# NVIDIA-Merlin/NVTabular

Measured on AMD Instinct MI355X. Metric: rows/sec + GB/s (Criteo Categorify+FillMissing+Normalize fit+transform, HBM-resident), higher is better.
Workload: dtype int32 keys -> int64 labels; fp64 moments/normalize; 1 GPU; synthetic Criteo-day0: 26 int32 categorical (Criteo-1TB cardinalities, Zipf) + 13 int32 continuous, nulls as Arrow bitmaps; Categorify + FillMissing + Normalize, fit + transform; rows_per_gpu=45000000, algorithmic_bytes_per_row=624, tie_break=value (count desc, value asc), artifacts=deferred (no parquet I/O inside the timed region)

## Files before the change

nvtabular_amd/csrc/nvt_encode.hip:

```cpp
#include <cstdlib>
#include <limits>
#include <type_traits>

#include "nvt_common.hpp"
#include "nvt_internal.hpp"
#include "nvt_prof.hpp"
#include "nvt_range.hpp"

namespace nvt {

template <typename K>
struct EncSlot;
template <>
struct EncSlot<int32_t> {
  int32_t key;
  int32_t label;
};
template <>
struct EncSlot<int64_t> {
  int64_t key;
  int64_t label;
};
template <typename K>
struct EncTraits;
// ... 20 lines not shown
  for (uint64_t i = (uint64_t)blockIdx.x * kBlock + threadIdx.x; i < capacity; i += stride)
    table[i] = e;
  if (blockIdx.x == 0 && threadIdx.x == 0) *sentinel_label = -1;
}

template <typename K>
__global__ __launch_bounds__(kBlock) void enc_build_kernel(const K *__restrict__ vocab, uint64_t n,
                                                           int64_t first_label, EncSlot<K> *table,
                                                           uint64_t mask, int64_t *sentinel_label) {
  constexpr K EMPTY = EncTraits<K>::empty;
  using C = typename EncTraits<K>::cas_t;
  const uint64_t stride = (uint64_t)gridDim.x * kBlock;
  for (uint64_t i = (uint64_t)blockIdx.x * kBlock + threadIdx.x; i < n; i += stride) {
    K key = vocab[i];
    int64_t label = first_label + (int64_t)i;
    if (key == EMPTY) {
      atomicMin(reinterpret_cast<unsigned long long *>(sentinel_label), (unsigned long long)label);
      continue;
    }
    uint64_t slot = (uint64_t)slot_hash(key) & mask;
    while (true) {
      K prev = (K)atomicCAS(reinterpret_cast<C *>(&table[slot].key), (C)EMPTY, (C)key);
      if (prev == EMPTY || prev == key) {
        using L = decltype(table[slot].label);
        if constexpr (sizeof(L) == 4)
          atomicMin(reinterpret_cast<int *>(&table[slot].label), (int)label);
        else
          atomicMin(reinterpret_cast<long long *>(&table[slot].label), (long long)label);
        break;
      }
      slot = (slot + 1) & mask;
    }
  }
}

__global__ __launch_bounds__(kBlock) void enc_build_unique_i32_kernel(
    const int32_t *__restrict__ vocab, uint64_t n, int64_t first_label, EncSlot<int32_t> *table,
    uint64_t mask, int64_t *sentinel_label) {
  const unsigned long long EMPTY_SLOT =
      ((unsigned long long)(uint32_t)std::numeric_limits<int32_t>::max() << 32) |
      (unsigned long long)(uint32_t)INT32_MIN;
  const uint64_t stride = (uint64_t)gridDim.x * kBlock;
  for (uint64_t i = (uint64_t)blockIdx.x * kBlock + threadIdx.x; i < n; i += stride) {
    int32_t key = vocab[i];
    int64_t label = first_label + (int64_t)i;
    if (key == INT32_MIN) {
      *sentinel_label = label;
      continue;
    }
    unsigned long long want = ((unsigned long long)(uint32_t)label << 32) | (uint32_t)key;
    uint64_t slot = (uint64_t)slot_hash(key) & mask;
    while (atomicCAS(reinterpret_cast<unsigned long long *>(&table[slot]), EMPTY_SLOT, want) !=
           EMPTY_SLOT)
      slot = (slot + 1) & mask;
  }
}

template <typename K>
__device__ __forceinline__ int64_t probe(const EncSlot<K> *__restrict__ table, uint64_t mask,
                                         K key) {
  constexpr K EMPTY = EncTraits<K>::empty;
  uint64_t slot = (uint64_t)slot_hash(key) & mask;
  while (true) {
    EncSlot<K> s = table[slot];
    if (s.key == key) return (int64_t)s.label;
    if (s.key == EMPTY) return -1;
    slot = (slot + 1) & mask;
  }
}

template <typename K, typename OUT>
__global__ __launch_bounds__(kBlock) void encode_kernel(
    const K *__restrict__ keys, const uint8_t *__restrict__ valid, uint64_t n,
    const EncSlot<K> *__restrict__ table, uint64_t mask, const int64_t *__restrict__ sentinel_label,
    int64_t null_label, int64_t oov_label, uint32_t num_buckets, OUT *__restrict__ out) {
  constexpr K EMPTY = EncTraits<K>::empty;
  constexpr int VEC = EncTraits<K>::vec;
  const int64_t sent = *sentinel_label;

  auto label_of = [&](K key, bool ok) -> OUT {
    if (!ok) return (OUT)null_label;
    int64_t lab = (key == EMPTY) ? sent : probe<K>(table, mask, key);
    if (lab < 0) {
      lab = oov_label;
      if (num_buckets > 1) lab += (int64_t)(key_hash32((int64_t)key) % num_buckets);
    }
    return (OUT)lab;
  };

  const uint64_t nvec = n / VEC;
  const uint64_t stride = (uint64_t)gridDim.x * kBlock;
  using VecT = typename std::conditional<sizeof(K) == 4, int4, longlong2>::type;
  const VecT *vkeys = reinterpret_cast<const VecT *>(keys);
  for (uint64_t v = (uint64_t)blockIdx.x * kBlock + threadIdx.x; v < nvec; v += stride) {
    VecT pack = vkeys[v];
    unsigned vbits = 0xF;
    if (valid != nullptr) {
      uint64_t row = v * VEC;
      vbits = (valid[row >> 3] >> (row & 7));
    }
    K k[VEC];
    if constexpr (sizeof(K) == 4) {
      k[0] = pack.x;
      k[1] = pack.y;
      k[2] = pack.z;
      k[3] = pack.w;
    } else {
      k[0] = pack.x;
      k[1] = pack.y;
    }
    OUT r[VEC];
#pragma unroll
    for (int j = 0; j < VEC; ++j) r[j] = label_of(k[j], (vbits >> j) & 1);
    OUT *dst = out + v * VEC;
    if constexpr (VEC * sizeof(OUT) == 32) {
      int4 a, b;
      memcpy(&a, &r[0], 16);
      memcpy(&b, &r[2], 16);
      reinterpret_cast<int4 *>(dst)[0] = a;
      reinterpret_cast<int4 *>(dst)[1] = b;
    } else if constexpr (VEC * sizeof(OUT) == 16) {
      int4 a;
      memcpy(&a, &r[0], 16);
      reinterpret_cast<int4 *>(dst)[0] = a;
    } else {
      int2 a;
      memcpy(&a, &r[0], 8);
      reinterpret_cast<int2 *>(dst)[0] = a;
    }
  }
  for (uint64_t i = nvec * VEC + (uint64_t)blockIdx.x * kBlock + threadIdx.x; i < n; i += stride)
    out[i] = label_of(keys[i], bit_valid(valid, i));
}

typedef int nvt_v4i __attribute__((ext_vector_type(4)));
template <typename V>
__device__ __forceinline__ V nt_load16(const V *p) {
  static_assert(sizeof(V) == 16, "16-byte vectors only");
  nvt_v4i r = __builtin_nontemporal_load(reinterpret_cast<const nvt_v4i *>(p));
  V v;
  memcpy(&v, &r, 16);
  return v;
}
template <typename V>
__device__ __forceinline__ void nt_store16(V v, V *p) {
  static_assert(sizeof(V) == 16, "16-byte vectors only");
  nvt_v4i r;
  memcpy(&r, &v, 16);
  __builtin_nontemporal_store(r, reinterpret_cast<nvt_v4i *>(p));
}
#ifndef NVT_HOT_DIV
#define NVT_HOT_DIV 4
#endif
constexpr int kEncBS = 1024;
template <typename K>
struct HotCfg;
template <>
struct HotCfg<int32_t> {
  static constexpr int slots = 16384;
};
template <>
struct HotCfg<int64_t> {
  static constexpr int slots = 8192;
};

constexpr int kHead16Buckets = 12288;
constexpr int kHead16Keys = kHead16Buckets * 2 / 8 * 7;
__device__ __forceinline__ void two_buckets16(int32_t key, uint32_t &b1, uint32_t &b2) {
  const uint32_t k = (uint32_t)key, lo = k ^ (k >> 7), hi = k >> 8;
  const uint32_t h1 = ((__umul24(hi, 0x5BD1E9u) + __umul24(lo, 0x9E3779u)) >> 17) & 0x7FFFu;
  const uint32_t h2 = ((__umul24(hi, 0x7FEB35u) + __umul24(lo, 0x846CA7u)) >> 17) & 0x7FFFu;
  b1 = (h1 + 2u * h1) >> 3;
  b2 = (h2 + 2u * h2) >> 3;
  b2 = b2 == b1 ? (b1 ^ 1u) : b2;
}
__device__ unsigned long long g_enc_stats[2];

template <int SLOTS, typename K>
__device__ __forceinline__ uint32_t lds_home(K key) {
  if constexpr (sizeof(K) == 4) {
    static_assert(SLOTS <= 16384, "14 index bits");
    return (mul24_hash((int32_t)key) >> 18) & (SLOTS - 1);
  } else {
    return (uint32_t)(slot_hash(key) >> 13) & (SLOTS - 1);
  }
}

struct HeadJob {
  const int32_t *keys;
  unsigned char *image;
  int64_t first_label;
  uint32_t n_hot;
};
constexpr int kHeadJobsMax = 32;
struct HeadJobs {
  HeadJob j[kHeadJobsMax];
};

template <typename K, bool TWO>
__device__ __forceinline__ void build_head(unsigned char *lraw, long long *s_sent_p,
                                           const K *__restrict__ hot_keys, uint32_t n_hot,
                                           int64_t first_label) {
  constexpr K EMPTY = EncTraits<K>::empty;
  constexpr int SLOTS = HotCfg<K>::slots;
  using L = decltype(EncSlot<K>::label);
  using C = typename EncTraits<K>::cas_t;
  EncSlot<K> *lt = reinterpret_cast<EncSlot<K> *>(lraw);
  int2 *tkeys = reinterpret_cast<int2 *>(lraw);
  uint32_t *tlab = reinterpret_cast<uint32_t *>(lraw + kHead16Buckets * 8);
  long long &s_sent = *s_sent_p;
  if constexpr (TWO) {
    for (int i = threadIdx.x; i < kHead16Buckets; i += kEncBS) {
      tkeys[i] = make_int2((int)EMPTY, (int)EMPTY);
      tlab[i] = 0u;
    }
  } else {
    for (int i = threadIdx.x; i < SLOTS; i += kEncBS) {
      lt[i].key = EMPTY;
      lt[i].label = 0;
    }
  }
  if (threadIdx.x == 0) s_sent = -1;
  __syncthreads();
  for (uint32_t i = threadIdx.x; i < n_hot; i += kEncBS) {
    K key = hot_keys[i];
    if (key == EMPTY) {
      s_sent = first_label + (long long)i;
      continue;
    }
    if constexpr (TWO) {
      uint32_t b1, b2;
      two_buckets16((int32_t)key, b1, b2);
      const uint32_t cand[4] = {2 * b1, 2 * b1 + 1, 2 * b2, 2 * b2 + 1};
      int *kw = reinterpret_cast<int *>(tkeys);
      unsigned short *lw = reinterpret_cast<unsigned short *>(tlab);
#pragma unroll
      for (int c = 0; c < 4; ++c) {
        const int prev = atomicCAS(&kw[cand[c]], (int)EMPTY, (int)key);
        if (prev == (int)EMPTY) {
          lw[cand[c]] = (unsigned short)i;
          break;
        }
      }
      continue;
    }
    uint32_t s = lds_home<SLOTS>(key);
    while (true) {
      K prev = (K)atomicCAS(reinterpret_cast<C *>(&lt[s].key), (C)EMPTY, (C)key);
      if (prev == EMPTY || prev == key) {
        if (prev == EMPTY) lt[s].label = (L)(first_label + (int64_t)i);
        break;
      }
      s = (s + 1) & (SLOTS - 1);
    }
  }
  __syncthreads();
}

template <typename K, bool TWO>
constexpr int kHeadLdsBytes = TWO ? kHead16Buckets * 12 : HotCfg<K>::slots * (int)sizeof(EncSlot<K>);

__global__ __launch_bounds__(kEncBS) void enc_head_build_many_kernel(HeadJobs jobs) {
  constexpr int kLdsBytes = kHeadLdsBytes<int32_t, true>;
  __shared__ __align__(16) unsigned char lraw[kLdsBytes];
  __shared__ long long s_sent;
  const HeadJob j = jobs.j[blockIdx.x];
  build_head<int32_t, true>(lraw, &s_sent, j.keys, j.n_hot, j.first_label);
  const int4 *src = reinterpret_cast<const int4 *>(lraw);
  int4 *dst = reinterpret_cast<int4 *>(j.image);
  for (int i = threadIdx.x; i < kLdsBytes / 16; i += kEncBS) dst[i] = src[i];
  if (threadIdx.x == 0) *reinterpret_cast<long long *>(j.image + kLdsBytes) = s_sent;
}

template <int SLOTS>
__global__ __launch_bounds__(kBlock) void encode_small_kernel(
    const int32_t *__restrict__ keys, const uint8_t *__restrict__ valid, uint64_t n, int64_t null_label,
    int64_t oov_label, uint32_t num_buckets, int64_t *__restrict__ out,
    const int32_t *__restrict__ hot_keys, uint32_t n_hot, int64_t first_label) {
  constexpr int32_t EMPTY = EncTraits<int32_t>::empty;
  __shared__ EncSlot<int32_t> lt[SLOTS];
  __shared__ long long s_sent;
  for (int i = threadIdx.x; i < SLOTS; i += kBlock) {
    lt[i].key = EMPTY;
    lt[i].label = 0;
  }
  if (threadIdx.x == 0) s_sent = -1;
  __syncthreads();
  for (uint32_t i = threadIdx.x; i < n_hot; i += kBlock) {
    const int32_t key = hot_keys[i];
    if (key == EMPTY) {
      s_sent = first_label + (long long)i;
      continue;
    }
    uint32_t sl = lds_home<SLOTS>(key);
    while (true) {
      const int32_t prev = atomicCAS(&lt[sl].key, EMPTY, key);
      if (prev == EMPTY || prev == key) {
        if (prev == EMPTY) lt[sl].label = (int32_t)(first_label + (int64_t)i);
        break;
      }
      sl = (sl + 1) & (SLOTS - 1);
    }
  }
  __syncthreads();
  const int64_t sent = (int64_t)s_sent;
  auto encode = [&](int32_t key, bool ok) -> int64_t {
    if (!ok) return null_label;
    int64_t lab = -1;
    if (key == EMPTY) {
      lab = sent;
    } else {
      uint32_t sl = lds_home<SLOTS>(key);
      while (true) {
        const EncSlot<int32_t> e = lt[sl];
        if (e.key == key) {
          lab = (int64_t)e.label;
          break;
        }
        if (e.key == EMPTY) break;
        sl = (sl + 1) & (SLOTS - 1);
      }
    }
    if (lab < 0) {
      lab = oov_label;
      if (num_buckets > 1) lab += (int64_t)(key_hash32((int64_t)key) % num_buckets);
    }
    return lab;
  };
  constexpr int RUN = 2 * kWave, U = 4;
  typedef int v2i_nt __attribute__((ext_vector_type(2)));
  const uint64_t stride = (uint64_t)gridDim.x * kBlock;
  const unsigned lane = threadIdx.x & (kWave - 1);
  const uint64_t nruns = n / RUN;
  const uint64_t wave = (uint64_t)blockIdx.x * (kBlock / kWave) +
                        (uint64_t)__builtin_amdgcn_readfirstlane(threadIdx.x / kWave);
  const uint64_t nwaves = stride / kWave;
  for (uint64_t r0 = wave * U; r0 < nruns; r0 += nwaves * U) {
    v2i_nt raw[U];
    unsigned vb[U];
#pragma unroll
    for (int u = 0; u < U; ++u) {
      raw[u] = v2i_nt{0, 0};
      vb[u] = 3u;
      if (r0 + u < nruns) {
        const uint64_t e = (r0 + u) * RUN + 2 * lane;
        raw[u] = __builtin_nontemporal_load(reinterpret_cast<const v2i_nt *>(keys + e));
        if (valid != nullptr) vb[u] = (unsigned)valid[e >> 3] >> (e & 7);
      }
    }
#pragma unroll
    for (int u = 0; u < U; ++u) {
      if (r0 + u >= nruns) break;
      const uint64_t e = (r0 + u) * RUN + 2 * lane;
      int64_t r[2];
      r[0] = encode(raw[u].x, (bool)(vb[u] & 1));
      r[1] = encode(raw[u].y, (bool)((vb[u] >> 1) & 1));
      nvt_v4i o;
      memcpy(&o, r, 16);
      __builtin_nontemporal_store(o, reinterpret_cast<nvt_v4i *>(out + e));
    }
  }
  for (uint64_t i = nruns * RUN + (uint64_t)blockIdx.x * kBlock + threadIdx.x; i < n; i += stride)
    out[i] = encode(keys[i], bit_valid(valid, i));
}

template <typename K, typename OUT, bool TWO = false, bool GLOBAL = true>
__global__ __launch_bounds__(kEncBS, 1) void encode_hot_kernel(
    const K *__restrict__ keys, const uint8_t *__restrict__ valid, uint64_t n,
    const EncSlot<K> *__restrict__ table, uint64_t mask, const int64_t *__restrict__ sentinel_label,
    int64_t null_label, int64_t oov_label, uint32_t num_buckets, OUT *__restrict__ out,
    const K *__restrict__ hot_keys, uint32_t n_hot, int64_t first_label, int count_stats = 0,
    const unsigned char *__restrict__ head_image = nullptr) {
  static_assert(!TWO || (GLOBAL && sizeof(K) == 4), "TWO: the 2-choice head of int32 keys in cache mode");
  constexpr bool global_needed = GLOBAL;
  constexpr K EMPTY = EncTraits<K>::empty;
  constexpr int VEC = EncTraits<K>::vec;
  constexpr int SLOTS = HotCfg<K>::slots;
  constexpr int kLdsBytes = kHeadLdsBytes<K, TWO>;
  __shared__ __align__(16) unsigned char lraw[kLdsBytes];
  EncSlot<K> *lt = reinterpret_cast<EncSlot<K> *>(lraw);
  int2 *tkeys = reinterpret_cast<int2 *>(lraw);
  uint32_t *tlab = reinterpret_cast<uint32_t *>(lraw + kHead16Buckets * 8);
  __shared__ long long s_sent;
  if (head_image != nullptr) {
    const int4 *src = reinterpret_cast<const int4 *>(head_image);
    int4 *dst = reinterpret_cast<int4 *>(lraw);
    for (int i = threadIdx.x; i < kLdsBytes / 16; i += kEncBS) dst[i] = src[i];
    if (threadIdx.x == 0) s_sent = *reinterpret_cast<const long long *>(head_image + kLdsBytes);
    __syncthreads();
  } else {
    build_head<K, TWO>(lraw, &s_sent, hot_keys, n_hot, first_label);
  }
  const int64_t sent = global_needed ? *sentinel_label : (int64_t)s_sent;

  auto hot_lookup = [&](K key) -> int64_t {
    if constexpr (TWO) {
      uint32_t b1, b2;
      two_buckets16((int32_t)key, b1, b2);
      const int2 a = tkeys[b1], c = tkeys[b2];
      const uint32_t la = tlab[b1], lc = tlab[b2];
      int lab = -1;
      lab = a.x == (int)key ? (int)(la & 0xFFFFu) : lab;
      lab = a.y == (int)key ? (int)(la >> 16) : lab;
      lab = c.x == (int)key ? (int)(lc & 0xFFFFu) : lab;
      lab = c.y == (int)key ? (int)(lc >> 16) : lab;
      return lab < 0 ? (int64_t)-1 : first_label + (int64_t)lab;
    }
    uint32_t s = lds_home<SLOTS>(key);
    while (true) {
      EncSlot<K> e = lt[s];
      if (e.key == key) return (int64_t)e.label;
      if (e.key == EMPTY) return -1;
      s = (s + 1) & (SLOTS - 1);
    }
  };
  auto finish = [&](K key, int64_t lab) -> OUT {
    if (lab < 0) {
      lab = oov_label;
      if (num_buckets > 1) lab += (int64_t)(key_hash32((int64_t)key) % num_buckets);
    }
    return (OUT)lab;
  };

  const uint64_t nvec = n / VEC;
  const uint64_t stride = (uint64_t)gridDim.x * kEncBS;
  using VecT = typename std::conditional<sizeof(K) == 4, int4, longlong2>::type;
  const VecT *vkeys = reinterpret_cast<const VecT *>(keys);
  constexpr int U = 2;
  constexpr int NK = U * VEC;
  VecT nxt_pack[U];
  unsigned nxt_vb[U];
  unsigned st_miss = 0, st_rows = 0;
  auto issue_loads = [&](uint64_t v0, VecT (&pk)[U], unsigned (&bits)[U]) {
#pragma unroll
    for (int u = 0; u < U; ++u) {
      uint64_t v = v0 + (uint64_t)u * stride;
      bits[u] = 0;
      if (v < nvec) {
        pk[u] = nt_load16(&vkeys[v]);
        bits[u] = 0x10000u | (valid ? (unsigned)valid[(v * VEC) >> 3] : 0xFFu);
      }
    }
  };
  issue_loads((uint64_t)blockIdx.x * kEncBS + threadIdx.x, nxt_pack, nxt_vb);
  for (uint64_t v0 = (uint64_t)blockIdx.x * kEncBS + threadIdx.x; v0 < nvec; v0 += stride * U) {
    VecT pack[U];
    unsigned vb[U];
#pragma unroll
    for (int u = 0; u < U; ++u) {
      pack[u] = nxt_pack[u];
      vb[u] = nxt_vb[u];
    }
    issue_loads(v0 + stride * U, nxt_pack, nxt_vb);
#pragma unroll
    for (int u = 0; u < U; ++u)
      if (vb[u])
        vb[u] = 0x100u | (((vb[u] & 0xFFu) >> (((v0 + (uint64_t)u * stride) * VEC) & 7)) &
                          ((1u << VEC) - 1u));
    K k[NK];
    int64_t lab[NK];
    bool need[NK];
#pragma unroll
    for (int u = 0; u < U; ++u) {
      if constexpr (sizeof(K) == 4) {
        k[u * VEC + 0] = pack[u].x;
        k[u * VEC + 1] = pack[u].y;
        k[u * VEC + 2] = pack[u].z;
        k[u * VEC + 3] = pack[u].w;
      } else {
        k[u * VEC + 0] = pack[u].x;
        k[u * VEC + 1] = pack[u].y;
      }
    }
#pragma unroll
    for (int q = 0; q < NK; ++q) {
      const bool ok = (vb[q / VEC] & 0x100) && ((vb[q / VEC] >> (q % VEC)) & 1);
      lab[q] = -1;
      need[q] = false;
      if (ok) {
        if (k[q] == EMPTY) {
          lab[q] = sent;
        } else {
          lab[q] = hot_lookup(k[q]);
          need[q] = lab[q] < 0 && global_needed;
          if (count_stats) {
            st_rows += 1u;
            st_miss += need[q] ? 1u : 0u;
          }
        }
      } else {
        lab[q] = null_label;
      }
    }
    if constexpr (GLOBAL) {
      uint64_t slot[NK];
      EncSlot<K> e[NK];
#pragma unroll
      for (int q = 0; q < NK; ++q) {
        slot[q] = (uint64_t)slot_hash(k[q]) & mask;
        if (need[q]) e[q] = table[slot[q]];
      }
#pragma unroll
      for (int q = 0; q < NK; ++q) {
        if (!need[q]) continue;
        while (true) {
          if (e[q].key == k[q]) {
            lab[q] = (int64_t)e[q].label;
            break;
          }
          if (e[q].key == EMPTY) break;
          slot[q] = (slot[q] + 1) & mask;
          e[q] = table[slot[q]];
        }
      }
    }
#pragma unroll
    for (int u = 0; u < U; ++u) {
      if (!(vb[u] & 0x100)) continue;
      uint64_t v = v0 + (uint64_t)u * stride;
      OUT r[VEC];
#pragma unroll
      for (int j = 0; j < VEC; ++j) {
        const int q = u * VEC + j;
        const bool ok = (vb[u] >> j) & 1;
        r[j] = ok ? finish(k[q], lab[q]) : (OUT)null_label;
      }
      OUT *dst = out + v * VEC;
      if constexpr (VEC * sizeof(OUT) == 32) {
        int4 a, b;
        memcpy(&a, &r[0], 16);
        memcpy(&b, &r[2], 16);
        nt_store16(a, &reinterpret_cast<int4 *>(dst)[0]);
        nt_store16(b, &reinterpret_cast<int4 *>(dst)[1]);
      } else if constexpr (VEC * sizeof(OUT) == 16) {
        int4 a;
        memcpy(&a, &r[0], 16);
        nt_store16(a, &reinterpret_cast<int4 *>(dst)[0]);
      } else {
        int2 a;
        memcpy(&a, &r[0], 8);
        reinterpret_cast<int2 *>(dst)[0] = a;
      }
    }
  }
  for (uint64_t i = nvec * VEC + (uint64_t)blockIdx.x * kEncBS + threadIdx.x; i < n; i += stride) {
    K key = keys[i];
    OUT r = (OUT)null_label;
    if (bit_valid(valid, i)) {
      int64_t lab = key == EMPTY ? sent : hot_lookup(key);
      if (lab < 0 && key != EMPTY && global_needed) {
        uint64_t sl = (uint64_t)slot_hash(key) & mask;
        while (true) {
          const EncSlot<K> e1 = table[sl];
          if (e1.key == key) {
            lab = (int64_t)e1.label;
            break;
          }
          if (e1.key == EMPTY) break;
          sl = (sl + 1) & mask;
        }
      }
      r = finish(key, lab);
    }
    out[i] = r;
  }
  if (count_stats) {
#pragma unroll
    for (int off = 32; off > 0; off >>= 1) {
      st_miss += __shfl_down(st_miss, off, 64);
      st_rows += __shfl_down(st_rows, off, 64);
    }
    if (lane_id() == 0) {
      atomicAdd(&g_enc_stats[0], (unsigned long long)st_miss);
      atomicAdd(&g_enc_stats[1], (unsigned long long)st_rows);
    }
  }
}

#define NVT_GLOBAL_AS __attribute__((address_space(1)))
template <typename T>
__device__ __forceinline__ NVT_GLOBAL_AS T *uniform_gptr(T *p) {
  const uint64_t v = reinterpret_cast<uint64_t>(p);
  const uint32_t lo = __builtin_amdgcn_readfirstlane((uint32_t)v);
  const uint32_t hi = __builtin_amdgcn_readfirstlane((uint32_t)(v >> 32));
  return (NVT_GLOBAL_AS T *)(((uint64_t)hi << 32) | lo);
}
template <typename OUT, int RANGE>
__global__ __launch_bounds__(kEncBS, 1) void encode_pipe_kernel(
    const int32_t *__restrict__ keys, const uint8_t *__restrict__ valid, uint64_t n,
    const EncSlot<int32_t> *__restrict__ table, uint64_t mask,
    const int64_t *__restrict__ sentinel_label, int64_t null_label, int64_t oov_label,
    uint32_t num_buckets, OUT *__restrict__ out, const int32_t *__restrict__ hot_keys,
    uint32_t n_hot, int64_t first_label, const int32_t *__restrict__ range_aux, int count_stats,
    const unsigned char *__restrict__ head_image) {
  static_assert(RANGE == 1 || RANGE == 2, "range tables (slots and byte offsets fit 32 bits)");
  using K = int32_t;
  constexpr K EMPTY = EncTraits<K>::empty;
  constexpr int VEC = 4, U = 2, NK = U * VEC;
  constexpr int kLdsBytes = kHeadLdsBytes<K, true>;
  RangeMap rmap = load_map(range_aux);
  __shared__ uint32_t s_pieces[RANGE == 1 ? kRpPwWords : 1];
  if constexpr (RANGE == 1) stage_pieces(rmap, s_pieces, threadIdx.x, kEncBS);
  __shared__ __align__(16) unsigned char lraw[kLdsBytes];
  const int2 *tkeys = reinterpret_cast<const int2 *>(lraw);
  const uint32_t *tlab = reinterpret_cast<const uint32_t *>(lraw + kHead16Buckets * 8);
  __shared__ long long s_sent;
  __shared__ unsigned s_next;
  if (threadIdx.x == 0) s_next = 0;
  if (head_image != nullptr) {
    const int4 *src = reinterpret_cast<const int4 *>(head_image);
    int4 *dst = reinterpret_cast<int4 *>(lraw);
    for (int i = threadIdx.x; i < kLdsBytes / 16; i += kEncBS) dst[i] = src[i];
    __syncthreads();
  } else {
    build_head<K, true>(lraw, &s_sent, hot_keys, n_hot, first_label);
  }
  const int32_t sent = (int32_t)*sentinel_label;
  const unsigned long long *tw = reinterpret_cast<const unsigned long long *>(table);
  const char *tbytes = reinterpret_cast<const char *>(table);

  unsigned st_miss = 0, st_rows = 0;
  auto run = [&](auto pw_tag) {
    constexpr bool PW = decltype(pw_tag)::value;
    auto first_slot = [&](K key) -> uint32_t {
      const uint32_t f = rmap.template fine_staged<PW>(key);
      return RANGE == 2 ? f : f + (f >> 14) * (uint32_t)kRpTail;
    };
    auto hot_lookup = [&](K key) -> int32_t {
      uint32_t b1, b2;
      two_buckets16(key, b1, b2);
      const int2 a = tkeys[b1], c = tkeys[b2];
      const uint32_t la = tlab[b1], lc = tlab[b2];
      int lab = -1;
      lab = a.x == key ? (int)(la & 0xFFFFu) : lab;
      lab = a.y == key ? (int)(la >> 16) : lab;
      lab = c.x == key ? (int)(lc & 0xFFFFu) : lab;
      lab = c.y == key ? (int)(lc >> 16) : lab;
      return lab < 0 ? -1 : (int32_t)first_label + lab;
    };
    auto walk = [&](K key, uint32_t sl0, unsigned long long e0) -> int32_t {
      if constexpr (RANGE == 2) {
        unsigned long long w = 0;
        const uint64_t at = flat_find_from(tw, mask + 1, (uint64_t)sl0, key, e0, &w);
        return at == ~0ull ? -1 : (int32_t)(w >> 32);
      } else {
        uint64_t sl = sl0;
        while (true) {
          const unsigned long long e = tw[++sl];
          if ((int32_t)(uint32_t)e == key) return (int32_t)(e >> 32);
          if ((int32_t)(uint32_t)e == EMPTY) return -1;
        }
      }
    };
    auto finish = [&](K key, int32_t lab) -> OUT {
      int64_t r = (int64_t)lab;
      if (lab < 0) {
        r = oov_label;
        if (num_buckets > 1) r += (int64_t)(key_hash32((int64_t)key) % num_buckets);
      }
      return (OUT)r;
    };
    auto encode_one = [&](K key, bool ok) -> OUT {
      if (!ok) return (OUT)null_label;
      int32_t lab = key == EMPTY ? sent : hot_lookup(key);
      if (lab < 0 && key != EMPTY) {
        const uint32_t sl = first_slot(key);
        const unsigned long long e = tw[sl];
        if ((int32_t)(uint32_t)e == key) lab = (int32_t)(e >> 32);
        else if ((int32_t)(uint32_t)e != EMPTY) lab = walk(key, sl, e);
      }
      return finish(key, lab);
    };

    const uint64_t nvec = n / VEC;
    const uint64_t stride = (uint64_t)gridDim.x * kEncBS, SU = stride * U;
    const uint64_t vb0 = (uint64_t)blockIdx.x * kEncBS;
    const int4 *vkeys = reinterpret_cast<const int4 *>(keys);
    const uint8_t *vsrc = valid != nullptr ? valid : reinterpret_cast<const uint8_t *>(keys);
    const unsigned vor = valid != nullptr ? 0u : 0xFFu;
    uint64_t nfull = 0;
    if (nvec >= vb0 + (uint64_t)(U - 1) * stride + kEncBS)
      nfull = (nvec - (vb0 + (uint64_t)(U - 1) * stride + kEncBS)) / SU + 1;
    const unsigned tid = threadIdx.x, lane = lane_id();
    const unsigned nib = (tid & 1u) * 4u;
    int4 nxt_pack[U];
    unsigned nxt_vb[U];
    struct Stage {
      int32_t k[NK];
      int32_t lab[NK];
      unsigned long long e[NK];
      unsigned need;
      unsigned vb[U];
    };
    auto batch_base = [&](uint64_t j, int u) -> uint64_t {
      return vb0 + (j >> 4) * SU + (uint64_t)u * stride + (j & 15u) * (uint64_t)kWave;
    };
    auto request_keys = [&](uint64_t j) {
#pragma unroll
      for (int u = 0; u < U; ++u) {
        const uint64_t vs = batch_base(j, u);
        const nvt_v4i raw = __builtin_nontemporal_load(
            reinterpret_cast<const NVT_GLOBAL_AS nvt_v4i *>(uniform_gptr(vkeys + vs)) + lane);
        nxt_pack[u] = make_int4(raw.x, raw.y, raw.z, raw.w);
        nxt_vb[u] = (unsigned)uniform_gptr(vsrc + (vs >> 1))[lane >> 1];
      }
    };
    auto lds_phase = [&](Stage &st) {
      unsigned need = 0;
#pragma unroll
      for (int u = 0; u < U; ++u) {
        st.k[u * VEC + 0] = nxt_pack[u].x;
        st.k[u * VEC + 1] = nxt_pack[u].y;
        st.k[u * VEC + 2] = nxt_pack[u].z;
        st.k[u * VEC + 3] = nxt_pack[u].w;
        st.vb[u] = ((nxt_vb[u] | vor) >> nib) & 0xFu;
      }
#pragma unroll
      for (int q = 0; q < NK; ++q) {
        const K key = st.k[q];
        const bool ok = (st.vb[q / VEC] >> (q % VEC)) & 1u;
        const bool is_sent = key == EMPTY;
        int32_t lab = hot_lookup(key);
        lab = is_sent ? sent : lab;
        st.lab[q] = lab;
        need |= ((ok & !is_sent & (lab < 0)) ? 1u : 0u) << q;
      }
      st.need = need;
      if (count_stats) {
        st_rows += (unsigned)__popc(st.vb[0]) + (unsigned)__popc(st.vb[1]);
        st_miss += (unsigned)__popc(need);
      }
    };
    auto request_probes = [&](Stage &st) {
#pragma unroll
      for (int q = 0; q < NK; ++q) {
        const uint32_t off = ((st.need >> q) & 1u) ? first_slot(st.k[q]) * 8u : 0u;
        st.e[q] = *reinterpret_cast<const unsigned long long *>(tbytes + off);
        if constexpr (PW) __builtin_amdgcn_sched_barrier(0);
      }
    };
    auto resolve = [&](Stage &st) {
      unsigned more = 0;
#pragma unroll
      for (int q = 0; q < NK; ++q) {
        const bool nd = (st.need >> q) & 1u;
        const int32_t ek = (int32_t)(uint32_t)st.e[q];
        const bool hit = nd & (ek == st.k[q]);
        st.lab[q] = hit ? (int32_t)(st.e[q] >> 32) : st.lab[q];
        more |= ((nd & !hit & (ek != EMPTY)) ? 1u : 0u) << q;
      }
      while (more) {
        const int q = (int)__ffs((int)more) - 1;
        more &= more - 1u;
        K key = st.k[0];
        unsigned long long e0 = st.e[0];
#pragma unroll
        for (int j = 1; j < NK; ++j) {
          key = q == j ? st.k[j] : key;
          e0 = q == j ? st.e[j] : e0;
        }
        const int32_t lab = walk(key, first_slot(key), e0);
#pragma unroll
        for (int j = 0; j < NK; ++j) st.lab[j] = q == j ? lab : st.lab[j];
      }
    };
    auto store = [&](const Stage &st, uint64_t j) {
#pragma unroll
      for (int u = 0; u < U; ++u) {
// ... 111 lines not shown
  if (count_stats) {
#pragma unroll
    for (int off = 32; off > 0; off >>= 1) {
      st_miss += __shfl_down(st_miss, off, 64);
      st_rows += __shfl_down(st_rows, off, 64);
    }
    if (lane_id() == 0) {
      atomicAdd(&g_enc_stats[0], (unsigned long long)st_miss);
      atomicAdd(&g_enc_stats[1], (unsigned long long)st_rows);
    }
  }
}

template <typename K>
__global__ __launch_bounds__(kBlock) void hash_bucket_kernel(const K *__restrict__ keys,
                                                             const uint8_t *__restrict__ valid,
                                                             uint64_t n, uint32_t nb,
                                                             int32_t *__restrict__ out,
                                                             const uint64_t *__restrict__ xor_in,
                                                             uint64_t *__restrict__ xor_out) {
  const uint64_t stride = (uint64_t)gridDim.x * kBlock;
  for (uint64_t i = (uint64_t)blockIdx.x * kBlock + threadIdx.x; i < n; i += stride) {
    uint64_t h = key_hash64(bit_valid(valid, i) ? (int64_t)keys[i] : 0);
    if (xor_in) h ^= xor_in[i];
    if (xor_out) xor_out[i] = h;
    if (out) out[i] = (int32_t)((uint32_t)(h >> 32) % nb);
  }
}

template <typename K>
__global__ __launch_bounds__(kBlock) void hash_bucket_vec_kernel(const K *__restrict__ keys,
                                                                 const uint8_t *__restrict__ valid,
                                                                 uint64_t n, uint32_t nb,
                                                                 int32_t *__restrict__ out) {
  constexpr int VEC = EncTraits<K>::vec;
  const uint64_t nvec = n / VEC;
  const uint64_t stride = (uint64_t)gridDim.x * kBlock;
  using VecT = typename std::conditional<sizeof(K) == 4, int4, longlong2>::type;
  const VecT *vkeys = reinterpret_cast<const VecT *>(keys);
  for (uint64_t v = (uint64_t)blockIdx.x * kBlock + threadIdx.x; v < nvec; v += stride) {
    VecT pack = vkeys[v];
    if (valid != nullptr) {
      const uint64_t row = v * VEC;
      const unsigned vb = (unsigned)valid[row >> 3] >> (row & 7);
      if (!(vb & 1)) pack.x = 0;
      if (!(vb & 2)) pack.y = 0;
      if constexpr (sizeof(K) == 4) {
        if (!(vb & 4)) pack.z = 0;
        if (!(vb & 8)) pack.w = 0;
      }
    }
    if constexpr (sizeof(K) == 4) {
      int4 r;
      r.x = (int32_t)(key_hash32(pack.x) % nb);
      r.y = (int32_t)(key_hash32(pack.y) % nb);
      r.z = (int32_t)(key_hash32(pack.z) % nb);
      r.w = (int32_t)(key_hash32(pack.w) % nb);
      reinterpret_cast<int4 *>(out)[v] = r;
    } else {
      int2 r;
      r.x = (int32_t)(key_hash32(pack.x) % nb);
      r.y = (int32_t)(key_hash32(pack.y) % nb);
      reinterpret_cast<int2 *>(out)[v] = r;
    }
  }
  for (uint64_t i = nvec * VEC + (uint64_t)blockIdx.x * kBlock + threadIdx.x; i < n; i += stride)
    out[i] = (int32_t)(key_hash32(bit_valid(valid, i) ? (int64_t)keys[i] : 0) % nb);
}

template <typename K>
int build_launch(const K *vocab, uint64_t n, int64_t first_label, void *table, uint64_t capacity,
                 int64_t *sentinel_label, int unique_keys, hipStream_t s) {
  NVT_CHECK_ARG(table && sentinel_label, "null table");
  NVT_CHECK_ARG(capacity >= 64 && (capacity & (capacity - 1)) == 0, "capacity must be 2^k >= 64");
  NVT_CHECK_ARG(capacity > n, "capacity must exceed the vocabulary size");
  NVT_CHECK_ARG(sizeof(K) == 8 || first_label + (int64_t)n < INT32_MAX, "labels overflow int32");
  NVT_CHECK_ARG(first_label >= 0, "first_label must not be negative");
  auto *t = reinterpret_cast<EncSlot<K> *>(table);
  NVT_PROF("encode_build", 0, s);
  enc_clear_kernel<K><<<stream_grid(capacity, kBlock * 4), kBlock, 0, s>>>(t, capacity,
                                                                           sentinel_label);
  NVT_CHECK_LAUNCH();
  if (n) {
    NVT_CHECK_ARG(vocab, "null vocabulary");
    if constexpr (sizeof(K) == 4) {
      if (unique_keys) {
        enc_build_unique_i32_kernel<<<stream_grid(n, kBlock), kBlock, 0, s>>>(
            vocab, n, first_label, t, capacity - 1, sentinel_label);
        NVT_CHECK_LAUNCH();
        return NVT_OK;
      }
    }
    enc_build_kernel<K><<<stream_grid(n, kBlock), kBlock, 0, s>>>(vocab, n, first_label, t,
                                                                  capacity - 1, sentinel_label);
    NVT_CHECK_LAUNCH();
  }
  return NVT_OK;
}

template <typename K>
int encode_launch(const K *keys, const uint8_t *valid, uint64_t n, const void *table,
                  uint64_t capacity, const int64_t *sentinel_label, int64_t null_label,
                  int64_t oov_label, uint32_t num_buckets, void *out, int out_bytes,
                  const K *hot_keys, uint64_t n_vocab, int64_t first_label, hipStream_t s,
                  const int32_t *range_aux = nullptr, const void *head_image = nullptr) {
  constexpr uint64_t kResident = sizeof(K) == 4 ? NVT_ENCODE_RESIDENT_I32 : NVT_ENCODE_RESIDENT_I64;
  const bool resident = hot_keys != nullptr && n_vocab > 0 && n_vocab <= kResident;
  NVT_CHECK_ARG(resident || (table && sentinel_label), "null table");
  NVT_CHECK_ARG(resident || range_aux || (capacity >= 64 && (capacity & (capacity - 1)) == 0),
                "capacity must be 2^k >= 64");
  NVT_CHECK_ARG(range_aux == nullptr || (sizeof(K) == 4 && hot_keys != nullptr && n_vocab > 0),
                "range tables: int32 keys with the ordered vocabulary (vocab_keys)");
  NVT_CHECK_ARG(out_bytes == 4 || out_bytes == 8, "out_bytes must be 4 or 8");
  if (n == 0) return NVT_OK;
  NVT_CHECK_ARG(keys && out, "null keys/out");
  NVT_CHECK_ARG((reinterpret_cast<uintptr_t>(keys) & 15) == 0 &&
                    (reinterpret_cast<uintptr_t>(out) & 15) == 0,
                "keys/out must be 16-byte aligned");
  constexpr int VEC = EncTraits<K>::vec;
  auto *t = reinterpret_cast<const EncSlot<K> *>(table);
  NVT_PROF(sizeof(K) == 4 ? "encode_i32" : "encode_i64", n * (sizeof(K) + (uint64_t)out_bytes), s);
  auto with_out = [&](auto launch) {
    if (out_bytes == 8) launch(reinterpret_cast<int64_t *>(out));
    else launch(reinterpret_cast<int32_t *>(out));
  };
  if (hot_keys != nullptr && n_vocab > 0) {
    const unsigned hgrid = stream_grid(n / VEC + 1, kEncBS * 2, 1);
    const uint64_t mask = capacity - 1;
    if (resident) {
      const uint32_t n_hot = (uint32_t)n_vocab;
      if constexpr (sizeof(K) == 4) {
        if (out_bytes == 8 && n_vocab <= 2048) {
          const unsigned sgrid = stream_grid(n / 2 + 1, kBlock * 8, 8);
          if (n_vocab <= 1024)
            encode_small_kernel<2048><<<sgrid, kBlock, 0, s>>>(
                keys, valid, n, null_label, oov_label, num_buckets, reinterpret_cast<int64_t *>(out),
                hot_keys, n_hot, first_label);
          else
            encode_small_kernel<4096><<<sgrid, kBlock, 0, s>>>(
                keys, valid, n, null_label, oov_label, num_buckets, reinterpret_cast<int64_t *>(out),
                hot_keys, n_hot, first_label);
          NVT_CHECK_LAUNCH();
          return NVT_OK;
        }
      }
      with_out([&](auto *o) {
        using OUT = std::remove_pointer_t<decltype(o)>;
        encode_hot_kernel<K, OUT, false, false><<<hgrid, kEncBS, 0, s>>>(
            keys, valid, n, t, mask, sentinel_label, null_label, oov_label, num_buckets, o, hot_keys,
            n_hot, first_label);
      });
    } else if constexpr (sizeof(K) == 4) {
      const uint32_t n_hot = (uint32_t)(n_vocab < (uint64_t)kHead16Keys ? n_vocab : (uint64_t)kHead16Keys);
      static const int stats = getenv("NVT_ENC_STATS") ? atoi(getenv("NVT_ENC_STATS")) : 0;
      const auto *image = reinterpret_cast<const unsigned char *>(head_image);
      with_out([&](auto *o) {
        using OUT = std::remove_pointer_t<decltype(o)>;
        if (range_aux == nullptr)
          encode_hot_kernel<K, OUT, true, true><<<hgrid, kEncBS, 0, s>>>(
              keys, valid, n, t, mask, sentinel_label, null_label, oov_label, num_buckets, o, hot_keys,
              n_hot, first_label, stats, image);
        else if (capacity > 0)
          encode_pipe_kernel<OUT, 2><<<hgrid, kEncBS, 0, s>>>(
              keys, valid, n, t, mask, sentinel_label, null_label, oov_label, num_buckets, o, hot_keys,
              n_hot, first_label, range_aux, stats, image);
        else
          encode_pipe_kernel<OUT, 1><<<hgrid, kEncBS, 0, s>>>(
              keys, valid, n, t, mask, sentinel_label, null_label, oov_label, num_buckets, o, hot_keys,
              n_hot, first_label, range_aux, stats, image);
      });
    } else {
      const uint32_t n_hot = (uint32_t)HotCfg<K>::slots / NVT_HOT_DIV;
      with_out([&](auto *o) {
        using OUT = std::remove_pointer_t<decltype(o)>;
        encode_hot_kernel<K, OUT, false, true><<<hgrid, kEncBS, 0, s>>>(
            keys, valid, n, t, mask, sentinel_label, null_label, oov_label, num_buckets, o, hot_keys,
            n_hot, first_label);
      });
    }
    NVT_CHECK_LAUNCH();
    return NVT_OK;
  }
  unsigned grid = stream_grid(n / VEC + 1, kBlock * 2, 8);
  if (out_bytes == 8)
    encode_kernel<K, int64_t><<<grid, kBlock, 0, s>>>(keys, valid, n, t, capacity - 1,
                                                      sentinel_label, null_label, oov_label,
                                                      num_buckets, reinterpret_cast<int64_t *>(out));
  else
    encode_kernel<K, int32_t><<<grid, kBlock, 0, s>>>(keys, valid, n, t, capacity - 1,
                                                      sentinel_label, null_label, oov_label,
                                                      num_buckets, reinterpret_cast<int32_t *>(out));
  NVT_CHECK_LAUNCH();
  return NVT_OK;
}

template <typename K>
int hash_bucket_launch(const K *keys, const uint8_t *valid, uint64_t n, uint32_t nb, int32_t *out,
                       const uint64_t *xor_in, uint64_t *xor_out, hipStream_t s) {
  NVT_CHECK_ARG(nb >= 1 && nb < (1u << 31), "num_buckets must be in [1, 2^31)");
  if (n == 0) return NVT_OK;
  NVT_CHECK_ARG(keys && (out || xor_out), "null keys/out");
  bool aligned = (reinterpret_cast<uintptr_t>(keys) & 15) == 0 &&
                 (reinterpret_cast<uintptr_t>(out) & 15) == 0;
  NVT_PROF("hash_bucket", n * (sizeof(K) + 4), s);
  if (!xor_in && !xor_out && aligned)
    hash_bucket_vec_kernel<K><<<stream_grid(n / EncTraits<K>::vec + 1, kBlock * 2), kBlock, 0, s>>>(
        keys, valid, n, nb, out);
  else
    hash_bucket_kernel<K><<<stream_grid(n, kBlock * 4), kBlock, 0, s>>>(keys, valid, n, nb, out,
                                                                       xor_in, xor_out);
  NVT_CHECK_LAUNCH();
  return NVT_OK;
}

int encode_build_any(int key_bytes, const void *vocab, uint64_t n, int64_t first_label, void *table,
                     uint64_t capacity, int64_t *sentinel_label, int unique_keys, hipStream_t s) {
  if (key_bytes == 4)
    return build_launch<int32_t>((const int32_t *)vocab, n, first_label, table, capacity,
                                 sentinel_label, unique_keys, s);
  return build_launch<int64_t>((const int64_t *)vocab, n, first_label, table, capacity,
                               sentinel_label, unique_keys, s);
}

int encode_clear_any(int key_bytes, void *table, uint64_t capacity, int64_t *sentinel_label,
                     hipStream_t s) {
  NVT_CHECK_ARG(table && sentinel_label, "null table");
  NVT_CHECK_ARG(capacity >= 64, "capacity must be >= 64");
  NVT_PROF("encode_build", 0, s);
  if (key_bytes == 4)
    enc_clear_kernel<int32_t><<<stream_grid(capacity, kBlock * 4), kBlock, 0, s>>>(
        reinterpret_cast<EncSlot<int32_t> *>(table), capacity, sentinel_label);
  else
    enc_clear_kernel<int64_t><<<stream_grid(capacity, kBlock * 4), kBlock, 0, s>>>(
        reinterpret_cast<EncSlot<int64_t> *>(table), capacity, sentinel_label);
  NVT_CHECK_LAUNCH();
  return NVT_OK;
}

int encode_insert_any(int key_bytes, const void *vocab, uint64_t n, int64_t first_label,
                      void *table, uint64_t capacity, int64_t *sentinel_label, hipStream_t s) {
  NVT_CHECK_ARG(key_bytes == 4, "encode_insert_any: int32 keys");
  NVT_CHECK_ARG(table && sentinel_label && (n == 0 || vocab), "null pointer");
  NVT_CHECK_ARG(first_label + (int64_t)n < INT32_MAX, "labels overflow int32");
  if (n == 0) return NVT_OK;
  NVT_PROF("encode_build", 0, s);
  enc_build_unique_i32_kernel<<<stream_grid(n, kBlock), kBlock, 0, s>>>(
      (const int32_t *)vocab, n, first_label, reinterpret_cast<EncSlot<int32_t> *>(table),
      capacity - 1, sentinel_label);
  NVT_CHECK_LAUNCH();
  return NVT_OK;
}

}

using namespace nvt;

namespace nvt {
int encode_head_build_many(const int32_t *const *vocab_keys, const uint64_t *n, const int64_t *first_label,
                           void *const *images, int count, hipStream_t s) {
  const uint64_t cap = (uint64_t)kHead16Keys;
  HeadJobs jobs;
  int m = 0;
  auto flush = [&]() -> int {
    if (m == 0) return NVT_OK;
    NVT_PROF("vocab_order", 0, s);
    enc_head_build_many_kernel<<<m, kEncBS, 0, s>>>(jobs);
    NVT_CHECK_LAUNCH();
    m = 0;
    return NVT_OK;
  };
  for (int i = 0; i < count; ++i) {
    if (images[i] == nullptr || vocab_keys[i] == nullptr || n[i] <= NVT_ENCODE_RESIDENT_I32) continue;
    jobs.j[m].keys = vocab_keys[i];
    jobs.j[m].image = (unsigned char *)images[i];
    jobs.j[m].first_label = first_label[i];
    jobs.j[m].n_hot = (uint32_t)(n[i] < cap ? n[i] : cap);
    if (++m == kHeadJobsMax) {
      int rc = flush();
      if (rc) return rc;
    }
  }
  return flush();
}
int encode_head_build(const int32_t *vocab_keys, uint64_t n, int64_t first_label, void *image,
                      hipStream_t s) {
  return encode_head_build_many(&vocab_keys, &n, &first_label, &image, 1, s);
}
}

extern "C" {

int nvt_encode_stats(uint64_t *out2, int reset, void *stream) {
  NVT_CHECK_ARG(out2, "null out");
  hipStream_t s = (hipStream_t)stream;
  NVT_CHECK_HIP(hipStreamSynchronize(s));
  unsigned long long v[2] = {0, 0};
  NVT_CHECK_HIP(hipMemcpyFromSymbol(v, HIP_SYMBOL(g_enc_stats), sizeof(v)));
  out2[0] = v[0];
  out2[1] = v[1];
  if (reset) {
    const unsigned long long z[2] = {0, 0};
    NVT_CHECK_HIP(hipMemcpyToSymbol(HIP_SYMBOL(g_enc_stats), z, sizeof(z)));
  }
  return NVT_OK;
}

int nvt_encode_table_bytes(int key_bytes, uint64_t capacity, uint64_t *bytes) {
  NVT_CHECK_ARG(bytes && (key_bytes == 4 || key_bytes == 8), "key_bytes must be 4 or 8");
  *bytes = capacity * (key_bytes == 4 ? sizeof(EncSlot<int32_t>) : sizeof(EncSlot<int64_t>));
  return NVT_OK;
}
int nvt_encode_build_i32(const int32_t *vocab_keys, uint64_t n_vocab, int64_t first_label,
                         void *table, uint64_t capacity, int64_t *sentinel_label, int unique_keys,
                         void *stream) {
  return build_launch<int32_t>(vocab_keys, n_vocab, first_label, table, capacity, sentinel_label,
                               unique_keys, (hipStream_t)stream);
}
int nvt_encode_build_i64(const int64_t *vocab_keys, uint64_t n_vocab, int64_t first_label,
                         void *table, uint64_t capacity, int64_t *sentinel_label, int unique_keys,
                         void *stream) {
  return build_launch<int64_t>(vocab_keys, n_vocab, first_label, table, capacity, sentinel_label,
                               unique_keys, (hipStream_t)stream);
}
int nvt_encode_i32(const int32_t *keys, const uint8_t *valid, uint64_t n, const void *table,
                   uint64_t capacity, const int64_t *sentinel_label, int64_t null_label,
                   int64_t oov_label, uint32_t num_buckets, void *out, int out_bytes,
                   const int32_t *vocab_keys, uint64_t n_vocab, int64_t first_label,
                   void *stream) {
  return encode_launch<int32_t>(keys, valid, n, table, capacity, sentinel_label, null_label,
                                oov_label, num_buckets, out, out_bytes, vocab_keys, n_vocab,
                                first_label, (hipStream_t)stream);
}
int nvt_encode_i64(const int64_t *keys, const uint8_t *valid, uint64_t n, const void *table,
                   uint64_t capacity, const int64_t *sentinel_label, int64_t null_label,
                   int64_t oov_label, uint32_t num_buckets, void *out, int out_bytes,
                   const int64_t *vocab_keys, uint64_t n_vocab, int64_t first_label,
                   void *stream) {
  return encode_launch<int64_t>(keys, valid, n, table, capacity, sentinel_label, null_label,
                                oov_label, num_buckets, out, out_bytes, vocab_keys, n_vocab,
                                first_label, (hipStream_t)stream);
}
int nvt_encode_many(const nvt_encode_col *cols, int ncols, void *stream) {
  NVT_CHECK_ARG(ncols == 0 || cols, "null descriptors");
  const int n_side = [] {
    const char *e = getenv("NVT_ENCODE_STREAMS");
    int v = e ? atoi(e) : 3;
    return v < 1 ? 1 : v > kSideStreams ? kSideStreams : v;
  }();
  hipStream_t main_s = (hipStream_t)stream;
  SidePool *pool = nullptr;
  const int lanes = ncols < n_side ? ncols : n_side;
  const bool fork = lanes > 1;
  if (fork) {
    int rc = side_pool(2, &pool);
    if (rc) return rc;
    NVT_CHECK_HIP(hipEventRecord(pool->fork, main_s));
    for (int k = 0; k < lanes; ++k) NVT_CHECK_HIP(hipStreamWaitEvent(pool->s[k], pool->fork, 0));
  }
  int rc_all = NVT_OK;
  for (int i = 0; i < ncols; ++i) {
    const nvt_encode_col &c = cols[i];
    hipStream_t cs = fork ? pool->s[i % lanes] : main_s;
    int rc;
    if (c.wait_event) NVT_CHECK_HIP(hipStreamWaitEvent(cs, (hipEvent_t)c.wait_event, 0));
    if (c.key_bytes == 4)
      rc = encode_launch<int32_t>((const int32_t *)c.keys, c.valid, c.n, c.table, c.capacity,
                                  c.sentinel_label, c.null_label, c.oov_label, c.num_buckets, c.out,
                                  c.out_bytes, (const int32_t *)c.vocab_keys, c.n_vocab,
                                  c.first_label, cs, c.range_aux, c.head_image);
    else if (c.key_bytes == 8)
      rc = encode_launch<int64_t>((const int64_t *)c.keys, c.valid, c.n, c.table, c.capacity,
                                  c.sentinel_label, c.null_label, c.oov_label, c.num_buckets, c.out,
                                  c.out_bytes, (const int64_t *)c.vocab_keys, c.n_vocab,
                                  c.first_label, cs);
    else {
      set_error("nvt_encode_many: key_bytes must be 4 or 8 (column %d)", i);
      rc = NVT_EINVAL;
    }
    if (rc) {
      rc_all = rc;
      break;
    }
  }
  if (fork)
    for (int k = 0; k < lanes; ++k) {
      NVT_CHECK_HIP(hipEventRecord(pool->join[k], pool->s[k]));
      NVT_CHECK_HIP(hipStreamWaitEvent(main_s, pool->join[k], 0));
    }
  return rc_all;
}
int nvt_hash_bucket_i32(const int32_t *keys, const uint8_t *valid, uint64_t n, uint32_t num_buckets,
                        int32_t *out, const uint64_t *xor_in, uint64_t *xor_out, void *stream) {
  return hash_bucket_launch<int32_t>(keys, valid, n, num_buckets, out, xor_in, xor_out,
                                     (hipStream_t)stream);
}
int nvt_hash_bucket_i64(const int64_t *keys, const uint8_t *valid, uint64_t n, uint32_t num_buckets,
                        int32_t *out, const uint64_t *xor_in, uint64_t *xor_out, void *stream) {
  return hash_bucket_launch<int64_t>(keys, valid, n, num_buckets, out, xor_in, xor_out,
                                     (hipStream_t)stream);
}

}
```

Measured before the change: 4.955 billion rows/s.

## Add cuckoo-kick head build and LDS-only encode when whole vocab fits head

When the whole vocabulary fits in the two-choice LDS head (no keys beyond the head), the head is built with cuckoo-style eviction kicks so every key gets placed. If no key is left unplaced, the encode kernels take a new path that looks up only the LDS table and skips the global hash-table probe and sentinel load. Any unplaced count is recorded in the head image so the fast path is only taken when the head is complete. This adds a random-walk insertion phase at build time and an extra image field, and leaves the fallback path unchanged for large vocabularies.

Result: faster. 5.041 billion rows/s (median of 5 runs) (+1.8%).

```diff
diff --git a/nvtabular_amd/csrc/nvt_encode.hip b/nvtabular_amd/csrc/nvt_encode.hip
--- a/nvtabular_amd/csrc/nvt_encode.hip
+++ b/nvtabular_amd/csrc/nvt_encode.hip
@@ -196,6 +196,9 @@
 #ifndef NVT_HOT_DIV
 #define NVT_HOT_DIV 4
 #endif
+#ifndef NVT_HEAD_KICKS
+#define NVT_HEAD_KICKS 256
+#endif
 constexpr int kEncBS = 1024;
 template <typename K>
 struct HotCfg;
@@ -235,16 +238,19 @@
   unsigned char *image;
   int64_t first_label;
   uint32_t n_hot;
+  uint32_t n_rest;
 };
 constexpr int kHeadJobsMax = 32;
 struct HeadJobs {
   HeadJob j[kHeadJobsMax];
 };
 
+constexpr int kHeadKicks = NVT_HEAD_KICKS;
 template <typename K, bool TWO>
 __device__ __forceinline__ void build_head(unsigned char *lraw, long long *s_sent_p,
                                            const K *__restrict__ hot_keys, uint32_t n_hot,
-                                           int64_t first_label) {
+                                           int64_t first_label, uint32_t n_rest = 1,
+                                           unsigned *s_unc_p = nullptr) {
   constexpr K EMPTY = EncTraits<K>::empty;
   constexpr int SLOTS = HotCfg<K>::slots;
   using L = decltype(EncSlot<K>::label);
@@ -254,6 +260,50 @@
   uint32_t *tlab = reinterpret_cast<uint32_t *>(lraw + kHead16Buckets * 8);
   long long &s_sent = *s_sent_p;
   if constexpr (TWO) {
+    if (threadIdx.x == 0) *s_unc_p = n_rest;
+    if (n_rest == 0) {
+      uint32_t *rw = reinterpret_cast<uint32_t *>(lraw);
+      for (int i = threadIdx.x; i < 2 * kHead16Buckets; i += kEncBS) rw[i] = 0u;
+      if (threadIdx.x == 0) s_sent = -1;
+      __syncthreads();
+      for (uint32_t i = threadIdx.x; i < n_hot; i += kEncBS) {
+        const int32_t key = (int32_t)hot_keys[i];
+        if (key == (int32_t)EMPTY) {
+          s_sent = first_label + (long long)i;
+          continue;
+        }
+        uint32_t b1, b2;
+        two_buckets16(key, b1, b2);
+        uint32_t hand = i + 1u;
+        const uint32_t cand[4] = {2 * b1, 2 * b1 + 1, 2 * b2, 2 * b2 + 1};
+#pragma unroll
+        for (int c = 0; c < 4; ++c)
+          if (hand && atomicCAS(&rw[cand[c]], 0u, hand) == 0u) hand = 0u;
+        uint32_t rnd = i * 2654435761u + 0x9E3779B9u;
+        uint32_t b = (rnd >> 16) & 1u ? b1 : b2;
+        for (int kick = 0; hand && kick < kHeadKicks; ++kick) {
+          rnd = rnd * 1664525u + 1013904223u;
+          const uint32_t old = atomicExch(&rw[2 * b + (rnd >> 31)], hand);
+          hand = old;
+          if (old == 0u) break;
+          two_buckets16((int32_t)hot_keys[old - 1u], b1, b2);
+          b = b == b1 ? b2 : b1;
+          if (atomicCAS(&rw[2 * b], 0u, hand) == 0u || atomicCAS(&rw[2 * b + 1], 0u, hand) == 0u)
+            hand = 0u;
+        }
+        if (hand) atomicAdd(s_unc_p, 1u);
+      }
+      __syncthreads();
+      int *kw = reinterpret_cast<int *>(tkeys);
+      unsigned short *lw = reinterpret_cast<unsigned short *>(tlab);
+      for (int i = threadIdx.x; i < 2 * kHead16Buckets; i += kEncBS) {
+        const uint32_t r = rw[i];
+        kw[i] = r ? (int)hot_keys[r - 1u] : (int)EMPTY;
+        lw[i] = (unsigned short)(r ? r - 1u : 0u);
+      }
+      __syncthreads();
+      return;
+    }
     for (int i = threadIdx.x; i < kHead16Buckets; i += kEncBS) {
       tkeys[i] = make_int2((int)EMPTY, (int)EMPTY);
       tlab[i] = 0u;
@@ -285,6 +335,7 @@
           lw[cand[c]] = (unsigned short)i;
           break;
         }
+        if (c == 3) atomicAdd(s_unc_p, 1u);
       }
       continue;
     }
@@ -308,12 +359,110 @@
   constexpr int kLdsBytes = kHeadLdsBytes<int32_t, true>;
   __shared__ __align__(16) unsigned char lraw[kLdsBytes];
   __shared__ long long s_sent;
+  __shared__ unsigned s_unc;
   const HeadJob j = jobs.j[blockIdx.x];
-  build_head<int32_t, true>(lraw, &s_sent, j.keys, j.n_hot, j.first_label);
+  build_head<int32_t, true>(lraw, &s_sent, j.keys, j.n_hot, j.first_label, j.n_rest, &s_unc);
   const int4 *src = reinterpret_cast<const int4 *>(lraw);
   int4 *dst = reinterpret_cast<int4 *>(j.image);
   for (int i = threadIdx.x; i < kLdsBytes / 16; i += kEncBS) dst[i] = src[i];
-  if (threadIdx.x == 0) *reinterpret_cast<long long *>(j.image + kLdsBytes) = s_sent;
+  if (threadIdx.x == 0) {
+    *reinterpret_cast<long long *>(j.image + kLdsBytes) = s_sent;
+    *reinterpret_cast<long long *>(j.image + kLdsBytes + 8) = (long long)s_unc;
+  }
+}
+
+template <typename OUT>
+__device__ __forceinline__ void encode_whole_head(
+    const int32_t *__restrict__ keys, const uint8_t *__restrict__ valid, uint64_t n,
+    const unsigned char *lraw, int32_t sent, int64_t null_label, int64_t oov_label, uint32_t num_buckets,
+    OUT *__restrict__ out, int64_t first_label, int count_stats) {
+  constexpr int32_t EMPTY = EncTraits<int32_t>::empty;
+  constexpr int KPL = 16 / (int)sizeof(OUT), RUN = KPL * kWave, U = 4;
+  typedef int kvec __attribute__((ext_vector_type(KPL)));
+  const int2 *tkeys = reinterpret_cast<const int2 *>(lraw);
+  const uint32_t *tlab = reinterpret_cast<const uint32_t *>(lraw + kHead16Buckets * 8);
+  auto encode = [&](int32_t key, bool ok) -> OUT {
+    if (!ok) return (OUT)null_label;
+    uint32_t b1, b2;
+    two_buckets16(key, b1, b2);
+    const int2 a = tkeys[b1], c = tkeys[b2];
+    const uint32_t la = tlab[b1], lc = tlab[b2];
+    int lab = -1;
+    lab = a.x == key ? (int)(la & 0xFFFFu) : lab;
+    lab = a.y == key ? (int)(la >> 16) : lab;
+    lab = c.x == key ? (int)(lc & 0xFFFFu) : lab;
+    lab = c.y == key ? (int)(lc >> 16) : lab;
+    lab = lab < 0 ? -1 : (int32_t)first_label + lab;
+    lab = key == EMPTY ? sent : lab;
+    int64_t r = (int64_t)lab;
+    if (lab < 0) {
+      r = oov_label;
+      if (num_buckets > 1) r += (int64_t)(key_hash32((int64_t)key) % num_buckets);
+    }
+    return (OUT)r;
+  };
+  const uint8_t *vsrc = valid != nullptr ? valid : reinterpret_cast<const uint8_t *>(keys);
+  const unsigned vor = valid != nullptr ? 0u : 0xFFu;
+  const unsigned lane = lane_id();
+  const unsigned sh = (KPL * lane) & 7u;
+  const uint64_t nruns = n / RUN;
+  const uint64_t wave = (uint64_t)blockIdx.x * (kEncBS / kWave) +
+                        (uint64_t)__builtin_amdgcn_readfirstlane(threadIdx.x / kWave);
+  const uint64_t step = (uint64_t)gridDim.x * (kEncBS / kWave) * U;
+  unsigned st_rows = 0;
+  auto one_run = [&](uint64_t r, kvec raw, unsigned vbyte) {
+    const unsigned bits = (vbyte | vor) >> sh;
+    OUT lab[KPL];
+#pragma unroll
+    for (int j = 0; j < KPL; ++j) lab[j] = encode(raw[j], (bits >> j) & 1u);
+    nvt_v4i o;
+    memcpy(&o, lab, 16);
+    __builtin_nontemporal_store(o, reinterpret_cast<nvt_v4i *>(out + r * RUN + KPL * lane));
+    if (count_stats) st_rows += (unsigned)__popc(bits & ((1u << KPL) - 1u));
+  };
+  uint64_t r0 = wave * U;
+  if (r0 + U <= nruns) {
+    kvec nxt[U];
+    unsigned nxt_vb[U];
+    auto request = [&](uint64_t at) {
+#pragma unroll
+      for (int u = 0; u < U; ++u) {
+        const uint64_t r = at + u < nruns ? at + u : nruns - 1;
+        const uint64_t e = r * RUN + KPL * lane;
+        nxt[u] = __builtin_nontemporal_load(reinterpret_cast<const kvec *>(keys + e));
+        nxt_vb[u] = (unsigned)vsrc[e >> 3];
+      }
+    };
+    request(r0);
+    for (; r0 + U <= nruns; r0 += step) {
+      kvec raw[U];
+      unsigned vb[U];
+#pragma unroll
+      for (int u = 0; u < U; ++u) {
+        raw[u] = nxt[u];
+        vb[u] = nxt_vb[u];
+      }
+      request(r0 + step);
+#pragma unroll
+      for (int u = 0; u < U; ++u) one_run(r0 + u, raw[u], vb[u]);
+    }
+  }
+  for (int u = 0; u < U; ++u) {
+    if (r0 + u >= nruns) break;
+    const uint64_t e = (r0 + u) * RUN + KPL * lane;
+    one_run(r0 + u, *reinterpret_cast<const kvec *>(keys + e), (unsigned)vsrc[e >> 3]);
+  }
+  for (uint64_t i = nruns * RUN + (uint64_t)blockIdx.x * kEncBS + threadIdx.x; i < n;
+       i += (uint64_t)gridDim.x * kEncBS) {
+    const bool ok = bit_valid(valid, i);
+    out[i] = encode(keys[i], ok);
+    if (count_stats) st_rows += ok ? 1u : 0u;
+  }
+  if (count_stats) {
+#pragma unroll
+    for (int off = 32; off > 0; off >>= 1) st_rows += __shfl_down(st_rows, off, 64);
+    if (lane == 0) atomicAdd(&g_enc_stats[1], (unsigned long long)st_rows);
+  }
 }
 
 template <int SLOTS>
@@ -414,7 +563,7 @@
     const EncSlot<K> *__restrict__ table, uint64_t mask, const int64_t *__restrict__ sentinel_label,
     int64_t null_label, int64_t oov_label, uint32_t num_buckets, OUT *__restrict__ out,
     const K *__restrict__ hot_keys, uint32_t n_hot, int64_t first_label, int count_stats = 0,
-    const unsigned char *__restrict__ head_image = nullptr) {
+    const unsigned char *__restrict__ head_image = nullptr, uint32_t n_rest = 1) {
   static_assert(!TWO || (GLOBAL && sizeof(K) == 4), "TWO: the 2-choice head of int32 keys in cache mode");
   constexpr bool global_needed = GLOBAL;
   constexpr K EMPTY = EncTraits<K>::empty;
@@ -426,14 +575,25 @@
   int2 *tkeys = reinterpret_cast<int2 *>(lraw);
   uint32_t *tlab = reinterpret_cast<uint32_t *>(lraw + kHead16Buckets * 8);
   __shared__ long long s_sent;
+  __shared__ unsigned s_unc;
   if (head_image != nullptr) {
     const int4 *src = reinterpret_cast<const int4 *>(head_image);
     int4 *dst = reinterpret_cast<int4 *>(lraw);
     for (int i = threadIdx.x; i < kLdsBytes / 16; i += kEncBS) dst[i] = src[i];
-    if (threadIdx.x == 0) s_sent = *reinterpret_cast<const long long *>(head_image + kLdsBytes);
+    if (threadIdx.x == 0) {
+      s_sent = *reinterpret_cast<const long long *>(head_image + kLdsBytes);
+      if constexpr (TWO) s_unc = *reinterpret_cast<const long long *>(head_image + kLdsBytes + 8) != 0;
+    }
     __syncthreads();
   } else {
-    build_head<K, TWO>(lraw, &s_sent, hot_keys, n_hot, first_label);
+    build_head<K, TWO>(lraw, &s_sent, hot_keys, n_hot, first_label, n_rest, &s_unc);
+  }
+  if constexpr (TWO) {
+    if (s_unc == 0) {
+      encode_whole_head<OUT>(keys, valid, n, lraw, (int32_t)s_sent, null_label, oov_label, num_buckets,
+                             out, first_label, count_stats);
+      return;
+    }
   }
   const int64_t sent = global_needed ? *sentinel_label : (int64_t)s_sent;
 
@@ -636,7 +796,7 @@
     const int64_t *__restrict__ sentinel_label, int64_t null_label, int64_t oov_label,
     uint32_t num_buckets, OUT *__restrict__ out, const int32_t *__restrict__ hot_keys,
     uint32_t n_hot, int64_t first_label, const int32_t *__restrict__ range_aux, int count_stats,
-    const unsigned char *__restrict__ head_image) {
+    const unsigned char *__restrict__ head_image, uint32_t n_rest) {
   static_assert(RANGE == 1 || RANGE == 2, "range tables (slots and byte offsets fit 32 bits)");
   using K = int32_t;
   constexpr K EMPTY = EncTraits<K>::empty;
@@ -650,14 +810,24 @@
   const uint32_t *tlab = reinterpret_cast<const uint32_t *>(lraw + kHead16Buckets * 8);
   __shared__ long long s_sent;
   __shared__ unsigned s_next;
+  __shared__ unsigned s_unc;
   if (threadIdx.x == 0) s_next = 0;
   if (head_image != nullptr) {
     const int4 *src = reinterpret_cast<const int4 *>(head_image);
     int4 *dst = reinterpret_cast<int4 *>(lraw);
     for (int i = threadIdx.x; i < kLdsBytes / 16; i += kEncBS) dst[i] = src[i];
+    if (threadIdx.x == 0) {
+      s_sent = *reinterpret_cast<const long long *>(head_image + kLdsBytes);
+      s_unc = *reinterpret_cast<const long long *>(head_image + kLdsBytes + 8) != 0;
+    }
     __syncthreads();
   } else {
-    build_head<K, true>(lraw, &s_sent, hot_keys, n_hot, first_label);
+    build_head<K, true>(lraw, &s_sent, hot_keys, n_hot, first_label, n_rest, &s_unc);
+  }
+  if (s_unc == 0) {
+    encode_whole_head<OUT>(keys, valid, n, lraw, (int32_t)s_sent, null_label, oov_label, num_buckets, out,
+                           first_label, count_stats);
+    return;
   }
   const int32_t sent = (int32_t)*sentinel_label;
   const unsigned long long *tw = reinterpret_cast<const unsigned long long *>(table);
@@ -1075,6 +1245,7 @@
       });
     } else if constexpr (sizeof(K) == 4) {
       const uint32_t n_hot = (uint32_t)(n_vocab < (uint64_t)kHead16Keys ? n_vocab : (uint64_t)kHead16Keys);
+      const uint32_t n_rest = (uint32_t)(n_vocab - n_hot);
       static const int stats = getenv("NVT_ENC_STATS") ? atoi(getenv("NVT_ENC_STATS")) : 0;
       const auto *image = reinterpret_cast<const unsigned char *>(head_image);
       with_out([&](auto *o) {
@@ -1082,15 +1253,15 @@
         if (range_aux == nullptr)
           encode_hot_kernel<K, OUT, true, true><<<hgrid, kEncBS, 0, s>>>(
               keys, valid, n, t, mask, sentinel_label, null_label, oov_label, num_buckets, o, hot_keys,
-              n_hot, first_label, stats, image);
+              n_hot, first_label, stats, image, n_rest);
         else if (capacity > 0)
           encode_pipe_kernel<OUT, 2><<<hgrid, kEncBS, 0, s>>>(
               keys, valid, n, t, mask, sentinel_label, null_label, oov_label, num_buckets, o, hot_keys,
-              n_hot, first_label, range_aux, stats, image);
+              n_hot, first_label, range_aux, stats, image, n_rest);
         else
           encode_pipe_kernel<OUT, 1><<<hgrid, kEncBS, 0, s>>>(
               keys, valid, n, t, mask, sentinel_label, null_label, oov_label, num_buckets, o, hot_keys,
-              n_hot, first_label, range_aux, stats, image);
+              n_hot, first_label, range_aux, stats, image, n_rest);
       });
     } else {
       const uint32_t n_hot = (uint32_t)HotCfg<K>::slots / NVT_HOT_DIV;
@@ -1198,6 +1369,7 @@
     jobs.j[m].image = (unsigned char *)images[i];
     jobs.j[m].first_label = first_label[i];
     jobs.j[m].n_hot = (uint32_t)(n[i] < cap ? n[i] : cap);
+    jobs.j[m].n_rest = (uint32_t)(n[i] - jobs.j[m].n_hot);
     if (++m == kHeadJobsMax) {
       int rc = flush();
       if (rc) return rc;
```
